# EnzoCording/FleetRL

Hardware: NVIDIA B200
Metric: EV-steps/sec (higher is better)
Workload: dtype f64

## Files before the change

fleetrl_b200/csrc/fleetstep.cu:

```cuda
#include <cuda_runtime.h>
#include <math.h>
#include <stdint.h>
#include <stdio.h>
#include <stdlib.h>
#include <string.h>

#include <string>
#include <vector>

#include "fleetstep.h"

namespace {

constexpr int kThreads = 256;
constexpr int kMinCtasPerSm = 4;
constexpr int kStatStripes = 64;
constexpr int kNQ = 5;
enum { Q_REWARD = 0, Q_CASH, Q_ATH, Q_MISS, Q_NVIOL };

constexpr uint32_t TF_TRIGGER = 1u;
constexpr uint32_t TF_LUNCH = 2u;

constexpr int EF_FROZEN = 1, EF_DONE = 2, EF_TRIGGER = 4, EF_LUNCH = 8, EF_RESET = 16;

// ... 166 lines not shown

template <bool kNorm, bool kAux>
__device__ __forceinline__ void write_ev_obs(const StepParams& p, float* __restrict__ o, int n, double soc, float hl,
                                             const EvRec& rec, bool flip) {
    const int N = p.N;
    o[n] = (float)soc;
    o[N + n] = kNorm ? (float)((double)hl / p.max_tl) : hl;
    if (kAux) {
        float4 ax = make_float4(rec.tt, rec.cl, rec.hn, rec.lax);
        if (flip) ax = aux_on_the_fly<kNorm>(0.9, rec.sr, rec.tl, rec.there, p.lc_batt_cap, p.hn_den, p.max_soc, p.max_hn);
        float* a = o + 2 * N + p.Ha;
        a[n] = (float)rec.there;
        a[N + n] = ax.x;
        a[2 * N + n] = ax.y;
        a[3 * N + n] = ax.z;
        a[4 * N + n] = ax.w;
    }
}

template <bool kAux>
__device__ __forceinline__ int hdr_pos(int Ha, int N, int q) {
    return q < Ha ? 2 * N + q : 2 * N + Ha + (kAux ? 5 * N : 0) + (q - Ha);
}
template <bool kAux>
__device__ __forceinline__ void copy_hdr(const StepParams& p, float* __restrict__ o, int n, int t) {
    const float* __restrict__ h = p.hdr + (size_t)t * p.hdr_stride;
    for (int q = n; q < (kAux ? p.Ha + p.Hb : p.Ha); q += p.N) o[hdr_pos<kAux>(p.Ha, p.N, q)] = __ldg(h + q);
}

template <bool kNorm, bool kAux>
__device__ __forceinline__ void reset_slot(const StepParams& p, int e, int n, int t0, float* obs_row, bool reinit_deg) {
    const size_t i = (size_t)e * p.N + n;
    const EvRec rec = load_rec(&p.ev_rec[(size_t)t0 * p.N + n]);
    bool flip = false;
    if (reinit_deg) {
        p.rf_len[i] = 1; p.fd_cyc[i] = 0; p.life[i] = 1 - p.init_soh;
        p.tflip[i] = 0;
    } else if (*p.n_flips != 0) {
        flip = p.tflip[i] != 0;
    }
    const double tgt = flip ? 0.9 : p.target;
    const double soh = 1.0 * p.init_soh;
    const double cap = soh * p.cap0;
    double soc = rec.sr;
    const float hl = rec.tl;
    const double time_needed = (tgt - soc) * cap / p.P;
    if (hl > 0.f && p.min_lax * time_needed > (double)hl) soc = tgt - (time_needed * p.P / cap) / p.min_lax;
    const double sdeg = (soc == 0) ? p.def_soc : soc;
    p.soc[i] = soc;
    p.hl[i] = hl;
    p.soh[i] = soh;
    p.hist[((size_t)e * p.R + 0) * p.N + n] = sdeg;
    if (p.rf_on) {
        const int slot = p.rf_ext[i];
        if (slot >= 0) { atomicExch(&p.ext_owner[slot], -1); p.rf_ext[i] = -1; }
        p.rf_stack[i * (size_t)p.rf_S] = sdeg;
        p.rf_dc[i] = 1u;
        p.rf_acc[i] = make_double2(0.0, 0.0);
    }
    if (obs_row) {
        write_ev_obs<kNorm, kAux>(p, obs_row, n, soc, hl, rec, flip);
        copy_hdr<kAux>(p, obs_row, n, t0);
    }
}

#ifdef POST_TIMING
__device__ unsigned long long g_post_clk[16];
#ifdef POST_TIMING_EVAL_ONLY
#define PT_ON(c_) (c_)
#else
#define PT_ON(c_) true
#endif
#define PT_START2(k_, c_) long long _pt = clock64(); const bool _pt_on = (k_) && PT_ON(c_)
#define PT_START(c_) PT_START2(true, c_)
#define PT_MARK(k) do { if (threadIdx.x == 0 && _pt_on) { const long long _c = clock64(); atomicAdd(&g_post_clk[k], (unsigned long long)(_c - _pt)); _pt = _c; } } while (0)
#define PT_COUNT(k, n) do { if (threadIdx.x == 0 && _pt_on) atomicAdd(&g_post_clk[k], (unsigned long long)(n)); } while (0)
#else
#define PT_START(c_) do {} while (0)
#define PT_START2(k_, c_) do {} while (0)
#define PT_MARK(k) do {} while (0)
#define PT_COUNT(k, n) do {} while (0)
#endif
constexpr int kPostThreads = 64;
constexpr int kRfBatch = 8;
constexpr int kRfQueue = 12;
constexpr int kRfPend = 8;
constexpr int kPostMinCtas = 8;

__device__ __forceinline__ double sei_cycle_stress(double range, double count, double mean, double s_temp) {
    const double k_sigma = 1.04, sigma_ref = 0.5, kd1 = 1.4E5, kd2 = -5.01E-1, kd3 = -1.23E5;
    double eff = range * count;
    eff = eff < 0 ? 0 : (eff > 1 ? 1 : eff);
    const double s_dod = 1.0 / (kd1 * exp(kd2 * log(eff)) + kd3);
    const double s_soc = exp(k_sigma * (mean - sigma_ref));
    return s_dod * s_soc * s_temp;
}

__global__ void debug_stress_kernel(const double* eff, const double* mean, double* out, int n) {
    const int i = blockIdx.x * blockDim.x + threadIdx.x;
    if (i < n) out[i] = sei_cycle_stress(eff[i], 1.0, mean[i], 1.0);
}

__device__ __noinline__ int rf_ext_alloc(const StepParams& p, size_t vid) {
    const unsigned P = (unsigned)p.rf_P;
    if (P == 0) return -1;
    unsigned q = (unsigned)(mix64((unsigned long long)vid) % P);
    for (unsigned k = 0; k < P; k++) {
        if (atomicCAS(&p.ext_owner[q], -1, (int)vid) == -1) return (int)q;
        if (++q == P) q = 0;
    }
    return -1;
}

__device__ __forceinline__ double empirical_eval(double dt, double evse, double old_soc, double new_soc) {
    const double avg_soc = (old_soc + new_soc) / 2;
    const double cs[3] = {0, 40, 90};
    const double ca[3] = {0.0065, 0.0293, 0.065};
    int best = 0;
    double bd = fabs(cs[0] - avg_soc);
#pragma unroll
    for (int k = 1; k < 3; k++) {
        const double d = fabs(cs[k] - avg_soc);
        if (d < bd) { bd = d; best = k; }
    }
    const double cal = ca[best] * dt / 8760;
    const double dod = fabs(new_soc - old_soc);
    const double cyc = (evse <= 22.0) ? dod * 0.000125 / 2 : dod * 0.000167 / 2;
    return cal + cyc;
}

__device__ __forceinline__ void cp_async_commit() { asm volatile("cp.async.commit_group;" ::: "memory"); }
template <int kPending>
__device__ __forceinline__ void cp_async_wait_group() { asm volatile("cp.async.wait_group %0;" :: "n"(kPending) : "memory"); }
__device__ __forceinline__ void cp_async4_hint(uint32_t sdst, const void* gsrc, uint64_t pol) {
    asm volatile("cp.async.ca.shared.global.L2::cache_hint [%0], [%1], 4, %2;" :: "r"(sdst), "l"(gsrc), "l"(pol) : "memory");
}
__device__ __forceinline__ void cp_async8_hint(uint32_t sdst, const void* gsrc, uint64_t pol) {
    asm volatile("cp.async.ca.shared.global.L2::cache_hint [%0], [%1], 8, %2;" :: "r"(sdst), "l"(gsrc), "l"(pol) : "memory");
}
__device__ __forceinline__ void cp_async16_hint(uint32_t sdst, const void* gsrc, uint64_t pol) {
    asm volatile("cp.async.cg.shared.global.L2::cache_hint [%0], [%1], 16, %2;" :: "r"(sdst), "l"(gsrc), "l"(pol) : "memory");
}
__device__ __forceinline__ uint64_t l2_evict_first_policy() {
    uint64_t pol;
    asm volatile("createpolicy.fractional.L2::evict_first.b64 %0, 1.0;" : "=l"(pol));
    return pol;
}

__device__ __forceinline__ double sei_fade_update(const StepParams& p, size_t i, int len, int m, int rfl, double msum,
                                                  double fsum, bool big, double s_temp, bool& consumed) {
    const double alpha_sei = 5.75E-2, beta_sei = 121, k_sigma = 1.04, sigma_ref = 0.5, k_dt = 4.14E-10;
    double deg = 0;
    consumed = false;
    p.n_cycles[i] = m;
    if (m > rfl) {
        const double battery_age = (double)(len - 1) * p.dt * 3600;
        const double mean_soc_cal = msum / (double)m;
        if (big) atomicOr(p.err_flags, 4u);
        const double fd_cal = (k_dt * battery_age) * exp(k_sigma * (mean_soc_cal - sigma_ref)) * s_temp;
        const double fd_cyc = p.fd_cyc[i] + fsum;
        p.fd_cyc[i] = fd_cyc;
        const double fd = fd_cyc + fd_cal;
        const double l_old = p.life[i];
        double new_l;
        if (p.init_soh == 1.0) {
            new_l = 1 - alpha_sei * exp(-beta_sei * fd) - (1 - alpha_sei) * exp(-fd);
            if (new_l < 0) atomicOr(p.err_flags, 2u);
        } else {
// ... 8 lines not shown
    p.soh[i] = p.soh[i] - deg;
    return deg;
}

__device__ __noinline__ double rf_vehicle_slow(const StepParams& p, int e, int n, int k_done, int k_now, bool evaluate,
                                               double s_temp) {
    const int N = p.N, S = p.rf_S, X = p.rf_X, Rm = p.Rm;
    const size_t i = (size_t)e * N + n;
    const unsigned int dc = p.rf_dc[i];
    int depth = (int)(dc & 0xffffu), c = (int)(dc >> 16);
    double2 acc = p.rf_acc[i];
    int slot = p.rf_ext[i];
    const int rfl = p.rf_len[i];
    const double* hcol = p.hist + (size_t)e * p.RN + n;
    double* stk = p.rf_stack + i * (size_t)S;
    double* ext = slot >= 0 ? p.ext_val + (size_t)slot * X : nullptr;
#define RF_GET(s_) ((s_) < S ? stk[(s_)] : ext[(s_) - S])
#define RF_PUT(s_, v_) do { if ((s_) < S) stk[(s_)] = (v_); else ext[(s_) - S] = (v_); } while (0)
    bool bad = false, big = false;
    double x_cur = hcol[(size_t)(k_done & Rm) * N];
    double dsg = x_cur - RF_GET(depth - 1);
    for (int r = k_done + 1; r <= k_now; r++) {
        const double x_next = hcol[(size_t)(r & Rm) * N];
        if (x_next == x_cur) continue;
        const double d = x_next - x_cur;
        if ((dsg < 0 && d > 0) || (dsg > 0 && d < 0)) {
            if (depth >= S && !ext) {
                slot = (depth < S + X) ? rf_ext_alloc(p, i) : -1;
                if (slot >= 0) ext = p.ext_val + (size_t)slot * X;
            }
            if (depth >= S + X || (depth >= S && !ext)) bad = true;
            else {
                RF_PUT(depth, x_cur); depth++;
                while (depth >= 3) {
                    const double x3 = RF_GET(depth - 1), x2 = RF_GET(depth - 2), x1 = RF_GET(depth - 3);
                    if (fabs(x3 - x2) < fabs(x2 - x1)) break;
                    const double range = fabs(x1 - x2), mean = 0.5 * (x1 + x2);
                    const bool half = depth == 3;
                    acc.x += mean;
                    if (c >= rfl - 1) { acc.y += sei_cycle_stress(range, half ? 0.5 : 1.0, mean, s_temp); big = big || range > 5; }
                    c++;
                    if (half) { RF_PUT(0, x2); RF_PUT(1, x3); depth = 2; }
                    else { RF_PUT(depth - 3, x3); depth -= 2; }
                }
            }
        }
        dsg = d; x_cur = x_next;
    }
    if (bad) atomicOr(p.err_flags, 8u);
    double deg = 0;
    if (evaluate) {
        const int len = k_now + 1;
        int m = c, h = depth, lo = 0;
        double msum = acc.x, fs = 0;
        if (len >= 3) {
            auto prov = [&](double xa, double xb, double cnt, bool last) {
                const double range = fabs(xa - xb), mean = 0.5 * (xa + xb);
                msum += mean;
                if (!last && m >= rfl - 1) { fs += sei_cycle_stress(range, cnt, mean, s_temp); big = big || range > 5; }
                m++;
            };
            while (h - lo >= 2) {
                const double x2 = RF_GET(h - 1), x1 = RF_GET(h - 2);
                if (fabs(x_cur - x2) < fabs(x2 - x1)) break;
                if (h - lo == 2) { prov(x1, x2, 0.5, false); lo++; }
                else { prov(x1, x2, 1.0, false); h -= 2; }
            }
            for (int k = lo; k + 1 < h; k++) prov(RF_GET(k), RF_GET(k + 1), 0.5, false);
            prov(RF_GET(h - 1), x_cur, 0.5, true);
        }
        bool consumed;
        deg = sei_fade_update(p, i, len, m, rfl, msum, acc.y + fs, big, s_temp, consumed);
        if (consumed) acc.y = 0;
    }
#undef RF_GET
#undef RF_PUT
    if (slot >= 0 && depth <= S) { atomicExch(&p.ext_owner[slot], -1); slot = -1; }
    p.rf_dc[i] = (unsigned int)depth | ((unsigned int)c << 16);
    p.rf_acc[i] = acc;
    p.rf_ext[i] = slot;
    return deg;
}

template <int kT, bool kEval>
__device__ __forceinline__ double rf_vehicle(const StepParams& p, int e, int n, bool active, int k_done, int k_now,
                                             bool evaluate, double s_temp, double* __restrict__ smcol,
                                             double* __restrict__ qcol, double2* __restrict__ pcol) {
    const unsigned full = 0xffffffffu;
    const int N = p.N, S = p.rf_S, Rm = p.Rm;
    const double inf = __longlong_as_double(0x7ff0000000000000ll);
    const size_t i = (size_t)e * N + (active ? n : 0);
    const double* __restrict__ hcol = p.hist + (size_t)e * p.RN + (active ? n : 0);
    double* __restrict__ stk = p.rf_stack + i * (size_t)S;
    int depth = 1, c = 0, rflm1 = 0;
    double2 acc = make_double2(0.0, 0.0);
    double x_cur = 0;
    if (active) {
        const unsigned int dc = p.rf_dc[i];
        acc = p.rf_acc[i];
        rflm1 = p.rf_len[i] - 1;
        x_cur = __ldcs(hcol + (size_t)(k_done & Rm) * N);
        for (int s = 0; s < S; s += 2) {
            const double2 v2 = *reinterpret_cast<const double2*>(stk + s);
            smcol[s * kT] = v2.x; smcol[(s + 1) * kT] = v2.y;
        }
        depth = (int)(dc & 0xffffu); c = (int)(dc >> 16);
    }
    bool slow = active && depth > S;
    bool live = active && !slow;
    PT_START2(kEval, evaluate);
    double t1 = 0, t2 = 0, Y = inf;
    if (live) {
        t1 = smcol[(depth - 1) * kT];
        if (depth >= 2) { t2 = smcol[(depth - 2) * kT]; Y = fabs(t1 - t2); }
    }
    double dsg = live ? x_cur - t1 : 0.0;
    bool big = false;
    int np = 0;
    bool has_item = false;
    double item_eff = 0, item_mean = 0;
#define RF_APPEND(target_)                                                                     \
    do {                                                                                       \
        if (has_item) { pcol[np * kT] = make_double2(item_eff, item_mean); np++; has_item = false; } \
        if (__any_sync(full, np == kRfPend)) RF_DRAIN(target_);                                \
    } while (0)
#define RF_DRAIN(target_)                                                                      \
    do {                                                                                       \
        const int m_ = __reduce_max_sync(full, np);                                            \
        for (int k_ = 0; k_ < m_; k_ += 2) {                                                   \
            const double2 i0_ = pcol[min(k_, kRfPend - 1) * kT];                     \
            const double2 i1_ = pcol[min(k_ + 1, kRfPend - 1) * kT];                 \
            const double s0_ = sei_cycle_stress(i0_.x, 1.0, i0_.y, s_temp);                    \
            const double s1_ = sei_cycle_stress(i1_.x, 1.0, i1_.y, s_temp);                    \
            if (k_ < np) (target_) += s0_;                                                     \
            if (k_ + 1 < np) (target_) += s1_;                                                 \
        }                                                                                      \
        np = 0;                                                                                \
    } while (0)

    int nq = 0;
    for (int r0 = k_done + 1; ; r0 += kRfBatch) {
        const bool more = r0 <= k_now;
        if (__any_sync(full, more ? nq > kRfQueue - kRfBatch : nq > 0)) {
            PT_MARK(2);
            int q = 0;
            while (__any_sync(full, q < nq)) {
                const bool act = q < nq;
                const double v = qcol[min(q, kRfQueue - 1) * kT];
                const double X = fabs(v - t1);
                const bool lt = X < Y, two = depth == 2;
                const bool closing = act && !lt;
                const bool full_c = closing && !two;
                const bool consume = act && (lt || two);
                const bool push = act && lt;
                if (push && depth >= S) { slow = true; live = false; nq = 0; }
                else {
                    const double mean = 0.5 * (t2 + t1);
                    acc.x += closing ? mean : 0.0;
                    has_item = closing && c >= rflm1;
                    item_eff = two ? 0.5 * Y : Y; item_mean = mean;
                    big = big || (closing && Y > 5);
                    c += closing ? 1 : 0;
                    if (push) smcol[max(depth - 2, 0) * kT] = t2;
                    depth += push ? 1 : (full_c ? -2 : 0);
                    const double s1 = smcol[max(depth - 1, 0) * kT], s2 = smcol[max(depth - 2, 0) * kT];
                    t2 = consume ? t1 : (full_c ? s2 : t2);
                    t1 = consume ? v : (full_c ? s1 : t1);
                    Y = consume ? X : (full_c ? (depth >= 2 ? fabs(t1 - t2) : inf) : Y);
                    q += consume ? 1 : 0;
                }
                PT_COUNT(10, 1);
                RF_APPEND(acc.y);
            }
            nq = 0;
            PT_MARK(3);
        }
        if (!__any_sync(full, more)) break;
        double xb[kRfBatch];
#pragma unroll
        for (int u = 0; u < kRfBatch; u++) xb[u] = __ldcs(hcol + (size_t)(min(r0 + u, k_now) & Rm) * N);
#pragma unroll
        for (int u = 0; u < kRfBatch; u++) {
            const double d = xb[u] - x_cur;
            const bool flip = live && (dsg * d < 0);
            if (flip) { qcol[nq * kT] = x_cur; nq++; }
            dsg = (d != 0) ? d : dsg;
            x_cur = live ? xb[u] : x_cur;
        }
    }
    RF_DRAIN(acc.y);
    PT_MARK(4);
    if (live) { smcol[(depth - 1) * kT] = t1; if (depth >= 2) smcol[(depth - 2) * kT] = t2; }

    double deg = 0;
    if (kEval && evaluate) {
        const int len = k_now + 1;
        int m = c, h = depth, lo = 0, k = 0;
        double msum = acc.x, fs = 0;
        int phase = (live && len >= 3) ? 0 : 2;
        while (__any_sync(full, phase < 2)) {
            if (phase == 0) {
                bool closed = false;
                if (h - lo >= 2) {
                    const double x2 = smcol[(h - 1) * kT], x1 = smcol[(h - 2) * kT];
                    const double yy = fabs(x2 - x1);
                    if (!(fabs(x_cur - x2) < yy)) {
                        closed = true;
                        const double mean = 0.5 * (x1 + x2);
                        msum += mean;
                        if (m >= rflm1) { has_item = true; item_eff = h - lo == 2 ? 0.5 * yy : yy; item_mean = mean; big = big || yy > 5; }
                        m++;
                        if (h - lo == 2) lo++; else h -= 2;
                    }
                }
                if (!closed) { phase = 1; k = lo; }
            } else if (phase == 1) {
                const double xa = smcol[k * kT], xb2 = (k + 1 < h) ? smcol[(k + 1) * kT] : x_cur;
                const double mean = 0.5 * (xa + xb2);
                msum += mean;
                if (k + 1 < h) {
                    const double rg = fabs(xa - xb2);
                    if (m >= rflm1) { has_item = true; item_eff = 0.5 * rg; item_mean = mean; big = big || rg > 5; }
                    k++;
                } else phase = 2;
                m++;
            }
            RF_APPEND(fs);
        }
        RF_DRAIN(fs);
        if (live) {
            bool consumed;
            deg = sei_fade_update(p, i, len, m, rflm1 + 1, msum, acc.y + fs, big, s_temp, consumed);
            if (consumed) acc.y = 0;
        }
    }
#undef RF_APPEND
#undef RF_DRAIN
    PT_MARK(5);
    if (live) {
        for (int s = 0; s < S; s += 2)
            *reinterpret_cast<double2*>(stk + s) = make_double2(smcol[s * kT], smcol[(s + 1) * kT]);
        p.rf_dc[i] = (unsigned int)depth | ((unsigned int)c << 16);
        p.rf_acc[i] = acc;
    }
    PT_MARK(6);
    if (slow) deg = rf_vehicle_slow(p, e, n, k_done, k_now, evaluate, s_temp);
    PT_MARK(7);
    return deg;
}

__device__ __forceinline__ void bulk_store_s2g(void* gdst, const void* ssrc, uint32_t bytes) {
    asm volatile("fence.proxy.async.shared::cta;" ::: "memory");
    asm volatile("cp.async.bulk.global.shared::cta.bulk_group [%0], [%1], %2;"
                 :: "l"(gdst), "r"((uint32_t)__cvta_generic_to_shared(ssrc)), "r"(bytes) : "memory");
    asm volatile("cp.async.bulk.commit_group;" ::: "memory");
}
__device__ __forceinline__ void bulk_store_s2g_nofence(void* gdst, const void* ssrc, uint32_t bytes) {
    uint64_t pol;
    asm volatile("createpolicy.fractional.L2::evict_first.b64 %0, 1.0;" : "=l"(pol));
    asm volatile("cp.async.bulk.global.shared::cta.bulk_group.L2::cache_hint [%0], [%1], %2, %3;"
                 :: "l"(gdst), "r"((uint32_t)__cvta_generic_to_shared(ssrc)), "r"(bytes), "l"(pol) : "memory");
    asm volatile("cp.async.bulk.commit_group;" ::: "memory");
}
__device__ __forceinline__ void thread_store_range(float* gdst, const float* ssrc, int nfl) {
    int head = (int)(((16u - (unsigned)((uintptr_t)gdst & 15u)) & 15u) >> 2);
    head = head < nfl ? head : nfl;
    const int mid = (nfl - head) & ~3;
    for (int k = 0; k < head; k++) gdst[k] = ssrc[k];
    if (mid > 0) bulk_store_s2g_nofence(gdst + head, ssrc + head, (uint32_t)mid * 4u);
    for (int k = head + mid; k < nfl; k++) gdst[k] = ssrc[k];
}
__device__ __forceinline__ void bulk_store_wait_read() {
    asm volatile("cp.async.bulk.wait_group.read 0;" ::: "memory");
}

__device__ __forceinline__ void ev_slot_step(const StepParams& p, const EnvS& es, size_t i, bool flip, double a, double soh,
                                             double sr, float ntl, int there, double& soc, float& hl, double& sdeg,
                                             double& q_rew, double& q_cash, double& q_ath, double& q_miss, double& q_nviol,
                                             double& q_en) {
    const double tgt = flip ? 0.9 : p.target;
    const double cap = soh * p.cap0;
    double c_cr = 0, c_dr = 0, c_inv = 0, c_oc = 0, c_dep = 0, c_cost = 0, c_rev = 0, c_miss = 0, c_nviol = 0;
    double num = 0;
    if (a >= 0) {
        const double dem = (tgt - soc) * cap;
        const double req = p.P * a * p.dt;
        if (req * p.eta_c > dem) {
            const double d = req - dem;
            const double pen = p.pen_oc * (d * d);
            c_oc = pen > p.clip_oc ? pen : p.clip_oc;
        }
        double en = 0;
        if (there == 1) en = fmin(dem / p.eta_c, req);
        else if (fabs(a) > 0.05) c_inv = p.pen_inv * (a * a);
        num = en * p.eta_c;
        q_en = en;
        double ge = en - es.pv_share;
        ge = ge > 0 ? ge : 0;
        c_cost = ge * es.S * p.mult;
        c_cr = es.F_cr * ge;
    } else if (a < 0) {
        const double left = -1 * soc * cap;
        const double req = p.P * a * p.dt;
        if (req * p.eta_d < left && there != 0) {
            const double d = left - req;
            c_oc = p.pen_oc * (d * d);
        }
        double en = 0.0;
        if (there == 1) en = fmax(left, req);
        else if (fabs(a) > 0.05) c_inv = p.pen_inv * (a * a);
        num = en;
        q_en = en;
        c_rev = -1 * en * es.Rfac;
        c_dr = es.F_dr * en;
    } else {
        q_en = 0;
        atomicOr(p.err_flags, 1u);
    }
    q_ath = a * (double)there;
    if (num != 0) soc = soc + num / cap;

    if (hl != 0.f && ntl == 0.f) {
        const double tg = (p.is_ct && (es.flags & EF_LUNCH)) ? p.target_lunch : tgt;
        const double diff = tg - soc;
// ... 516 lines not shown
        PF_MARK(7);
#endif

        double q_rew = 0, q_cash = 0, q_ath = 0, q_miss = 0, q_nviol = 0;
        double o_soc = 0, o_sdeg = 0, o_en = 0;
        float o_hl = 0.f;
        size_t o_hist = 0;
        if (active) {
            const EnvS& es = envs[b];
            float* orow = obs_tile + b * D;
            const size_t i = (size_t)tile * cstride + j;
            const int t1 = min(es.t + 1, p.T - 1);
            const int k = es.t - es.t_start;
            const EvRec rec = decode_rec(reinterpret_cast<const int4*>(stp + kPfStR0)[j],
                                         reinterpret_cast<const int4*>(stp + kPfStR1)[j]);
            o_soc = reinterpret_cast<const double*>(stp + kPfStSoc)[j];
            o_sdeg = reinterpret_cast<const double*>(stp + kPfStSdeg)[j];
            const double soh = reinterpret_cast<const double*>(stp + kPfStSoh)[j];
            o_hl = reinterpret_cast<const float*>(stp + kPfStHl)[j];
            const double a = (double)reinterpret_cast<const float*>(stp + kPfStA32)[j];
            float hv0 = 0.f;
            if (n < H) hv0 = reinterpret_cast<const float*>(stp + kPfStHv)[j];
            const bool flip = s_have_flips && p.tflip[i] != 0;
            ev_slot_step(p, es, i, flip, a, soh, rec.sr, rec.tl, rec.there_prev, o_soc, o_hl, o_sdeg, q_rew, q_cash, q_ath,
                         q_miss, q_nviol, o_en);
            o_hist = (size_t)(unsigned)tile * p.pf_tile_hist + hist_slot + (unsigned)(((k + 1) & p.Rm) * N);
            write_ev_obs<kNorm, kAux>(p, orow, n, o_soc, o_hl, rec, flip);
            if (n < H) orow[hpos] = hv0;
            for (int q = n + N; q < H; q += N)
                orow[hdr_pos<kAux>(p.Ha, N, q)] = ld_keep_f32(p.hdr + (size_t)t1 * p.hdr_stride + q, keep);
        }
        if (pair) {
            q_rew += __shfl_xor_sync(0xffffffffu, q_rew, 1);
            q_cash += __shfl_xor_sync(0xffffffffu, q_cash, 1);
            q_ath += __shfl_xor_sync(0xffffffffu, q_ath, 1);
            q_miss += __shfl_xor_sync(0xffffffffu, q_miss, 1);
            q_nviol += __shfl_xor_sync(0xffffffffu, q_nviol, 1);
        }
        if (active && !(pair && (j & 1))) {
            const int cj = pair ? (j >> 1) : j;
            contrib[Q_REWARD * cslots + cj] = q_rew;
            contrib[Q_CASH * cslots + cj] = q_cash;
            contrib[Q_ATH * cslots + cj] = q_ath;
            contrib[Q_MISS * cslots + cj] = q_miss;
            contrib[Q_NVIOL * cslots + cj] = q_nviol;
        }
        PF_MARK(1);
        asm volatile("fence.proxy.async.shared::cta;" ::: "memory");
        mbar_arrive(&bar_done[buf]);
        PF_MARK(5);
        PF_TRACE(tid >> 5, it, 3);
        if (active) {
            const size_t i = (size_t)tile * cstride + j;
            __stcs(p.soc + i, o_soc);
            __stcs(p.hl + i, o_hl);
            __stcs(p.hist + o_hist, o_sdeg);
            if (kLog) __stcs(p.charge_log + i, o_en);
        }
        PF_MARK(6);
        issue_copies(tile + kPfStages * G, ev_next, stg);
        PF_MARK(3);
        PF_TRACE(tid >> 5, it, 4);
        if (++stg == kPfStages) stg = 0;
        if (++ebuf == kPfEnvs) { ebuf = 0; ph_env ^= 1u; }
        if (++buf == kPfOut) { buf = 0; if (it >= kPfOut) ph_free ^= 1u; }
    }
    PF_FLUSH(8);
}

__device__ __forceinline__ void post_finish_lists(const StepParams& p) {
    if (threadIdx.x == 0) {
        __threadfence();
        const unsigned int d = atomicAdd(p.wl_done, 1u);
        if (d == gridDim.x - 1) {
            p.wl_count[0] = 0; p.wl_count[1] = 0; p.wl_count[2] = 0; p.wl_count[3] = 0; p.wl_count[4] = 0;
            *p.wl_done = 0;
        }
    }
}

template <bool kNorm, bool kAux, int kT>
__global__ void __launch_bounds__(kT, kT == 32 ? 2 * kPostMinCtas : kPostMinCtas) fleet_post_kernel(const __grid_constant__ StepParams p) {
    extern __shared__ __align__(16) unsigned char smem_raw[];
    double* sm_stack = reinterpret_cast<double*>(smem_raw);
    double* sm_queue = sm_stack + (size_t)p.rf_S * kT;
    double2* sm_pend = reinterpret_cast<double2*>(sm_queue + (size_t)kRfQueue * kT);
    __shared__ int s_w;
    __shared__ int2 s_ent;
    __shared__ int4 s_ev;
    __shared__ double s_deg;
    const int tid = threadIdx.x, N = p.N;
    const int n_front = p.wl_count[0];
    const int count = n_front + p.wl_count[2];
    const double temp_ref = 25, k_temp = 6.93E-2;
    const double s_temp = exp(k_temp * (p.temperature - temp_ref) * ((temp_ref + 273.15) / (p.temperature + 273.15)));

    const int chunks = p.post_chunks, cv = p.post_cv;
    const int items = count * chunks;
    if (tid == 0) {
        s_w = blockIdx.x; s_deg = 0;
        if (s_w < items) { s_ent = wl_fetch(p, s_w / chunks, n_front); s_ev = p.env4[s_ent.x]; }
    }
    for (;;) {
        __syncthreads();
        const int item = s_w;
        if (item >= items) break;
        const int w = item / chunks, chunk = item - w * chunks;
        const int2 ent = s_ent;
        const int e = ent.x, wf = ent.y;
        const int4 ev = s_ev;
        const int k_now = ev.x - ev.y;
        const int n = chunk * cv + tid;
        const bool mine = tid < cv && n < N;
        int w_next = 0;
        int2 ent_next = make_int2(0, 0);
        int4 ev_next = make_int4(0, 0, 0, 0);
        if (tid == 0) {
            w_next = atomicAdd(p.wl_count + 1, 1) + (int)gridDim.x;
            if (w_next < items) { ent_next = wl_fetch(p, w_next / chunks, n_front); ev_next = p.env4[ent_next.x]; }
        }
        PT_START((wf & WL_TRIGGER) != 0);
        PT_COUNT(11, 1);
        if (p.rf_on && (wf & (WL_TRIGGER | WL_FLUSH))) {
            PT_COUNT(12, 1);
            const double deg = rf_vehicle<kT, true>(p, e, n, mine, ev.w, k_now, (wf & WL_TRIGGER) != 0, s_temp, sm_stack + tid,
                                              sm_queue + tid, sm_pend + tid);
            if (deg != 0) atomicAdd(&s_deg, deg);
        } else if ((wf & WL_TRIGGER) && mine) {
            const double* hbase = p.hist + (size_t)e * p.RN;
            const size_t ii = (size_t)e * N + n;
            double deg = 0;
            if (k_now >= 1) deg = empirical_eval(p.dt, p.evse, hbase[(size_t)((k_now - 1) & p.Rm) * N + n], hbase[(size_t)(k_now & p.Rm) * N + n]);
            p.n_cycles[ii] = 0;
            p.last_deg[ii] = deg;
            p.soh[ii] = p.soh[ii] - deg;
            if (deg != 0) atomicAdd(&s_deg, deg);
        }
        __syncthreads();
        PT_MARK(8);
        if (tid == 0 && s_deg != 0)
            atomicAdd(p.stats + (size_t)(w % kStatStripes) * FLEET_S__COUNT + FLEET_S_DEGRADATION, s_deg);
        int t0 = 0;
        if (wf & WL_RESET) {
            PT_COUNT(13, 1);
            t0 = episode_start(p, p.next_start, e, ev.z);
            if (mine) reset_slot<kNorm, kAux>(p, e, n, t0, p.obs ? p.obs + (size_t)e * p.D : nullptr, !p.carry);
            PT_MARK(14);
        }
        if (tid == 0) {
            bool last = true;
            if (chunks > 1) {
                __threadfence();
                last = atomicAdd(p.wl_chunks + w, 1) == chunks - 1;
                if (last) p.wl_chunks[w] = 0;
            }
            if (last) {
                if (wf & WL_RESET) {
                    begin_episode(p, e, t0, ev.z);
                } else if (p.rf_on) {
                    p.env4[e] = make_int4(ev.x, ev.y, ev.z, k_now);
                }
            }
        }
        __syncthreads();
        PT_MARK(9);
        if (tid == 0) { s_w = w_next; s_ent = ent_next; s_ev = ev_next; s_deg = 0; }
    }

    const int n_flush = p.wl_count[3];
    if (n_flush > 0) {
        const unsigned full = 0xffffffffu;
        const int lane = tid & 31;
        const int vehicles = n_flush * N;
        const int units = (vehicles + 31) >> 5;
        for (;;) {
            int u = 0;
            if (lane == 0) u = atomicAdd(p.wl_count + 4, 1);
            u = __shfl_sync(full, u, 0);
            if (u >= units) break;
#ifdef POST_TIMING
            const long long pt_u = clock64();
#endif
            const int v = (u << 5) + lane;
            const bool active = v < vehicles;
            int4 fe = make_int4(0, 0, 0, 0);
            int n = 0;
            if (active) {
                const int f = v / N;
                n = v - f * N;
                fe = p.wl_flush[f];
            }
            if (active && n == N - 1) p.env4[fe.x].w = fe.z;
            rf_vehicle<kT, false>(p, fe.x, n, active, fe.y, fe.z, false, s_temp, sm_stack + tid, sm_queue + tid, sm_pend + tid);
#ifdef POST_TIMING
            if (lane == 0) { atomicAdd(&g_post_clk[15], 1ull); atomicAdd(&g_post_clk[0], (unsigned long long)(clock64() - pt_u)); }
#endif
        }
    }
    __syncthreads();
    post_finish_lists(p);
}

template <bool kNorm, bool kAux>
__global__ void __launch_bounds__(kThreads) fleet_reset_kernel(const StepParams p) {
    const int N = p.N, B = p.B;
    const int e0 = blockIdx.x * B;
    const int nb = min(B, p.E - e0);
    const int nslots = nb * N;
    for (int j = threadIdx.x; j < nslots; j += kThreads) {
        const int b = j / N, n = j - b * N;
        const int e = e0 + b;
        if (p.mask && !p.mask[e]) continue;
        const int t0 = episode_start(p, p.start_idx, e, p.env4[e].z);
        reset_slot<kNorm, kAux>(p, e, n, t0, p.obs ? p.obs + (size_t)e * p.D : nullptr, !p.carry);
    }
    __syncthreads();
    if (threadIdx.x < nb) {
        const int e = e0 + threadIdx.x;
        if (!(p.mask && !p.mask[e])) {
            const int ep_count = p.env4[e].z;
            begin_episode(p, e, episode_start(p, p.start_idx, e, ep_count), ep_count);
        }
    }
}

__global__ void init_state_kernel(StepParams p) {
    const size_t i = (size_t)blockIdx.x * blockDim.x + threadIdx.x;
    const size_t EN = (size_t)p.E * p.N;
    if (i < EN) {
        p.soc[i] = 0; p.hl[i] = 0; p.soh[i] = p.init_soh;
        p.rf_len[i] = 1; p.fd_cyc[i] = 0; p.life[i] = 1 - p.init_soh; p.n_cycles[i] = 0; p.last_deg[i] = 0;
        p.tflip[i] = 0;
        if (p.rf_on) { p.rf_dc[i] = 1u; p.rf_acc[i] = make_double2(0.0, 0.0); p.rf_ext[i] = -1; }
    }
    if (i < (size_t)p.E) p.env4[i] = make_int4(0, 0, 0, 0);
}

__global__ void policy_kernel(StepParams p, int policy, int ch_hour, int ch_minute, int max_h, const uint16_t* __restrict__ tod,
                              const int2* __restrict__ st_in, int2* __restrict__ st_out, float* __restrict__ actions) {
    const size_t i = (size_t)blockIdx.x * blockDim.x + threadIdx.x;
    if (i >= (size_t)p.E * p.N) return;
    const int e = (int)(i / p.N), n = (int)(i - (size_t)e * p.N);
    const int t = min(p.env4[e].x, p.T - 1);
    float a = 1.f;
    if (policy != FLEET_POLICY_UNCONTROLLED) {
        const EvRec rec = load_rec(&p.ev_rec[(size_t)t * p.N + n]);
        const bool flip = (*p.n_flips != 0) && p.tflip[i] != 0;
        const double tgt = flip ? 0.9 : p.target;
        const double cl = tgt * (double)rec.there - rec.sr;
        const double hn = cl * p.lc_batt_cap / p.hn_den;
        double d = hn / ((double)rec.tl + 0.001);
        d = d < 0 ? 0 : (d > 1 ? 1 : d);
        if (policy == FLEET_POLICY_DISTRIBUTED) {
            a = (float)d;
        } else {
            const int hour = tod[t] / 60, minute = tod[t] % 60;
            int2 st = st_in[e];
            if (p.is_ct && hour >= 11 && hour <= 14) {
                a = (float)d;
            } else {
                if ((ch_hour <= hour && ch_minute <= minute) || st.x) {
                    if (!st.x) st.y = t;
                    st.x = 1;
                    a = 1.f;
                } else {
                    a = 0.f;
                }
                if (st.x && (double)(t - st.y) * p.dt > (double)max_h) st.x = 0;
            }
            if (n == 0) st_out[e] = st;
        }
    }
    actions[i] = a;
}

__global__ void gather_field_kernel(StepParams p, int field, void* dst) {
// ... 590 lines not shown
        rfX = env_int("FLEETSTEP_RF_EXT", 52);
        if (rfS + rfX > c.episode_steps + 1) rfX = c.episode_steps + 1 - rfS;
        if (rfX < 0) rfX = 0;
        rfP = rfX > 0 ? env_int("FLEETSTEP_RF_EXT_SLOTS", (int)(EN / 128 < 64 ? 64 : (EN / 128 > (1u << 20) ? (1u << 20) : EN / 128))) : 0;
        if (EN >= 0x7fffffffull) return fail(h, FLEET_E_INVALID, "num_envs * num_evs must be below 2^31");
    }
    if ((rc = dev_alloc(h, &p.env4, (size_t)E))) return rc;
    if ((rc = dev_alloc(h, &p.soc, EN))) return rc;
    if ((rc = dev_alloc(h, &p.hl, EN))) return rc;
    if ((rc = dev_alloc(h, &p.soh, EN))) return rc;
    if ((rc = dev_alloc(h, &p.hist, EN * (size_t)R))) return rc;
    if ((rc = dev_alloc(h, &p.tflip, EN))) return rc;
    if ((rc = dev_alloc(h, &p.n_flips, (size_t)4))) return rc;
    if ((rc = dev_alloc(h, &p.env_f64, (size_t)EF__COUNT * E))) return rc;
    if ((rc = dev_alloc(h, &p.rf_len, EN))) return rc;
    if ((rc = dev_alloc(h, &p.fd_cyc, EN))) return rc;
    if ((rc = dev_alloc(h, &p.life, EN))) return rc;
    if ((rc = dev_alloc(h, &p.n_cycles, EN))) return rc;
    if ((rc = dev_alloc(h, &p.last_deg, EN))) return rc;
    if ((rc = dev_alloc(h, &p.stats, (size_t)kStatStripes * FLEET_S__COUNT))) return rc;
    if ((rc = dev_alloc(h, &p.err_flags, (size_t)4))) return rc;
    if ((rc = dev_alloc(h, &p.wl, (size_t)E))) return rc;
    if ((rc = dev_alloc(h, &p.wl_flush, (size_t)E))) return rc;
    if (rf_on) {
        if ((rc = dev_alloc(h, &p.rf_stack, EN * (size_t)rfS))) return rc;
        if ((rc = dev_alloc(h, &p.rf_dc, EN))) return rc;
        if ((rc = dev_alloc(h, &p.rf_acc, EN))) return rc;
        if ((rc = dev_alloc(h, &p.rf_ext, EN))) return rc;
        if ((rc = dev_alloc(h, &p.ext_owner, (size_t)(rfP > 0 ? rfP : 1)))) return rc;
        if ((rc = dev_alloc(h, &p.ext_val, (size_t)(rfP > 0 ? rfP : 1) * (size_t)(rfX > 0 ? rfX : 1), false))) return rc;
        CUDA_TRY(h, cudaMemset(p.ext_owner, 0xff, sizeof(int) * (size_t)(rfP > 0 ? rfP : 1)));
    }
    if ((rc = dev_alloc(h, &p.wl_count, (size_t)8))) return rc;
    if ((rc = dev_alloc(h, &p.wl_done, (size_t)4))) return rc;

    p.rf_on = rf_on ? 1 : 0; p.rf_S = rfS; p.rf_X = rfX; p.rf_P = rfP;
    p.E = E; p.N = N; p.T = T; p.R = R; p.Rm = R - 1; p.L = c.episode_steps; p.D = h->D; p.Ha = Ha; p.Hb = Hb; p.hdr_stride = hdr_stride;
    p.B = N >= kThreads ? 1 : kThreads / N;
    p.RN = (unsigned long long)R * (unsigned long long)N;
    p.is_ct = c.is_caretaker; p.calc_deg = c.calc_degradation; p.deg_mode = c.deg_mode; p.carry = c.carry_degradation_state;
    p.auto_reset = c.auto_reset; p.start_lo = c.start_lo; p.start_hi = c.start_hi; p.seed = c.seed;
    p.env_id_offset = env_id_offset;
    p.dt = c.dt; p.dt_f = (float)c.dt;
    p.P = c.obc_max_power < c.evse_max_power ? c.obc_max_power : c.evse_max_power;
    p.eta_c = c.charging_eff; p.eta_d = c.discharging_eff; p.mult = c.variable_multiplier; p.cap0 = c.init_battery_cap;
    p.target = 1.0 * c.target_soc; p.target_lunch = c.target_soc_lunch; p.eps = c.soc_eps; p.def_soc = c.def_soc;
    p.min_lax = c.min_laxity; p.pen_inv = c.penalty_invalid_action; p.pen_oc = c.penalty_overcharging;
    p.clip_oc = c.clip_overcharging; p.pen_ovl = c.penalty_overloading; p.full_reward = c.fully_charged_reward;
    p.evse = c.evse_max_power; p.grid = c.grid_connection; p.init_soh = c.init_soh; p.lc_batt_cap = c.lc_batt_cap;
    p.hn_den = c.evse_max_power * c.charging_eff;
    p.price_mult = c.price_multiplier; p.temperature = c.temperature;
    p.max_tl = c.max_time_left; p.max_soc = c.target_soc;
    p.max_hn = (c.target_soc * c.init_battery_cap) / (c.evse_max_power * c.charging_eff);
    p.ev_rec = d_rec; p.step_row = d_rows; p.hdr = d_hdr;
    {
        std::vector<uint16_t> tod((size_t)T);
        for (int tt = 0; tt < T; tt++) tod[tt] = (uint16_t)(tb->hour[tt] * 60 + tb->minute[tt]);
        if ((rc = dev_alloc(h, &h->tod, (size_t)T, false))) return rc;
        CUDA_TRY(h, cudaMemcpy(h->tod, tod.data(), tod.size() * sizeof(uint16_t), cudaMemcpyHostToDevice));
    }

    p.n_magic = (unsigned int)((0x100000000ull + (unsigned long long)N - 1) / (unsigned long long)N);
    {
        const unsigned long long Hh = (unsigned long long)(Ha + Hb > 0 ? Ha + Hb : 1);
        p.h_magic = (unsigned int)((0x100000000ull + Hh - 1) / Hh);
    }
    p.off_contrib = (int)smem_envs_bytes(p.B);
    p.off_obs = (int)smem_obs_offset(p.B, N);
    p.bulk_ok = ((p.B * h->D) % 4 == 0) ? 1 : 0;

    size_t sm = smem_step_bytes(p.B, N, h->D);
    if ((int64_t)sm > (int64_t)h->max_smem_optin) {
        char buf[256];
        snprintf(buf, sizeof buf, "step kernel needs %zu bytes of shared memory (N=%d, D=%d) but the device allows %d", sm, N,
                 h->D, h->max_smem_optin);
        return fail(h, FLEET_E_INVALID, buf);
    }
    h->num_sms = prop.multiProcessorCount;
    h->need_post = (c.calc_degradation || c.auto_reset) ? 1 : 0;
    h->post_threads = N <= 32 ? 32 : 64;
    p.post_chunks = (N + h->post_threads - 1) / h->post_threads;
    p.post_cv = (N + p.post_chunks - 1) / p.post_chunks;
    if (p.post_chunks > 1 && (rc = dev_alloc(h, &p.wl_chunks, (size_t)E))) return rc;
    h->smem_post = align16((size_t)(rfS + kRfQueue + 2 * kRfPend) * h->post_threads * 8);
    if ((int64_t)h->smem_post > (int64_t)h->max_smem_optin) return fail(h, FLEET_E_INVALID, "rf_stack_depth does not fit the post kernel's shared memory");
    {
        int per_sm = 1;
        CUDA_TRY(h, cudaFuncSetAttribute(pick_post(h), cudaFuncAttributeMaxDynamicSharedMemorySize, (int)h->smem_post));
        CUDA_TRY(h, cudaOccupancyMaxActiveBlocksPerMultiprocessor(&per_sm, pick_post(h), h->post_threads, h->smem_post));
        if (per_sm < 1) per_sm = 1;
        const int64_t g = (int64_t)h->num_sms * per_sm;
        h->grid_post = (int)(g < E ? g : E);
        const int cap = env_int("FLEETSTEP_POST_GRID", 0);
        if (cap > 0 && cap < h->grid_post) h->grid_post = cap;
    }
    h->smem_step = sm;
    {
        const char* zc = getenv("FLEETSTEP_HOST_ZEROCOPY");
        h->host_zerocopy = (zc && atoi(zc) == 0) ? 0 : 1;
    }
    {
        const char* force = getenv("FLEETSTEP_KERNEL");
        const bool want = !force || strcmp(force, "pf") == 0;
        const int pfB = kPfSlots / N;
        if (want && c.auto_reset && N >= 8 && pfB >= 1 && pfB <= 32) {
            const size_t smpf = pf_smem_bytes(pfB, N, h->D);
            int per_sm = 0;
            if ((int64_t)smpf <= (int64_t)h->max_smem_optin &&
                cudaFuncSetAttribute(pick_pf(h, false), cudaFuncAttributeMaxDynamicSharedMemorySize, (int)smpf) == cudaSuccess &&
                cudaFuncSetAttribute(pick_pf(h, true), cudaFuncAttributeMaxDynamicSharedMemorySize, (int)smpf) == cudaSuccess &&
                cudaOccupancyMaxActiveBlocksPerMultiprocessor(&per_sm, pick_pf(h, true), kPfThreads, smpf) == cudaSuccess && per_sm >= 1) {
                h->smem_pf = smpf;
                const int ntiles = (E + pfB - 1) / pfB;
                p.pf_B = pfB;
                p.pf_bulk = 1;
                p.pf_ntiles = ntiles;
                p.pf_tile_hist = (unsigned int)((size_t)pfB * p.RN);
                p.pf_pair = (N & 1) ? 0 : 1;
                p.pf_cslots = pf_contrib_slots(pfB, N);
                p.pf_cper = p.pf_pair ? N / 2 : N;
                p.pf_envs_b = (int)align16((size_t)pfB * sizeof(EnvS));
                p.pf_contrib_b = (int)align16((size_t)kNQ * p.pf_cslots * 8);
                p.pf_obs_b = (int)align16((size_t)pfB * h->D * 4 + 12);
                p.pf_off_contrib = kPfEnvs * p.pf_envs_b;
                p.pf_off_sums = p.pf_off_contrib + kPfOut * p.pf_contrib_b;
                p.pf_off_obs = p.pf_off_sums + 2 * (int)align16((size_t)kNQ * pfB * 8);
                p.pf_off_stage = (int)align16((size_t)p.pf_off_obs + (size_t)kPfOut * p.pf_obs_b);
                const int g = prop.multiProcessorCount * per_sm;
                h->grid_pf = g < ntiles ? g : ntiles;
                const int cap = env_int("FLEETSTEP_PF_GRID", 0);
                if (cap > 0 && cap < h->grid_pf) h->grid_pf = cap;
                h->use_pf = 1;
            }
            cudaGetLastError();
        }
        if (force && strcmp(force, "pf") == 0 && !h->use_pf)
            return fail(h, FLEET_E_INVALID, "FLEETSTEP_KERNEL=pf requested but the configuration does not qualify (needs auto_reset, 8 <= N <= 256)");
    }
    h->grid = (E + p.B - 1) / p.B;
    CUDA_TRY(h, cudaFuncSetAttribute(pick_step(h), cudaFuncAttributeMaxDynamicSharedMemorySize, (int)sm));

    init_state_kernel<<<(unsigned)((EN > (size_t)E ? EN : (size_t)E) + 255) / 256, 256>>>(p);
    h->launches++;
    CUDA_TRY(h, cudaGetLastError());
    CUDA_TRY(h, cudaDeviceSynchronize());
    return FLEET_OK;
}

int fleet_reset(FleetHandle* h, const int32_t* start_idx_dev, const uint8_t* mask_dev, float* obs_dev, void* stream) {
    if (!h) return FLEET_E_INVALID;
    CUDA_TRY(h, cudaSetDevice(h->device));
    StepParams p = h->p;
    p.start_idx = start_idx_dev; p.mask = mask_dev; p.obs = obs_dev;
    pick_reset(h)<<<h->grid, kThreads, 0, (cudaStream_t)stream>>>(p);
    h->launches++;
    if (h->log_n) fleet_log_launch(h, p, 1, (cudaStream_t)stream);
    CUDA_TRY(h, cudaGetLastError());
    return FLEET_OK;
}

int fleet_step(FleetHandle* h, const float* actions_dev, float* obs_dev, float* reward_dev, uint8_t* done_dev,
               float* terminal_obs_dev, void* stream) {
    if (!h) return FLEET_E_INVALID;
    if (!actions_dev) return fail(h, FLEET_E_INVALID, "actions_dev is NULL");
    CUDA_TRY(h, cudaSetDevice(h->device));
    StepParams p = h->p;
    p.actions = actions_dev; p.obs = obs_dev; p.reward = reward_dev; p.done = done_dev; p.terminal_obs = terminal_obs_dev;
// ... 203 lines not shown
```

Baseline: 24.59 billion.

## Stream rainflow history spans via cp.async and prefetch next flush work unit

Rainflow processing now loads the vehicle's stack and up to 16 history rows into shared memory with cp.async and an L2 evict-first hint, instead of strided direct loads in batches of 8. Turning-point detection runs over the shared span, and the detected points reuse the span buffer in place of a separate queue. Stack entries are stored as double2 with lookahead reads of the next stack values. In the flush loop, the next work-unit claim and its metadata fetch overlap the current vehicle's async loads through a pre-wait callback. This restructures the memory schedule and adds complexity, and the larger span buffer raises shared-memory use and can lower occupancy.

```diff
diff --git a/fleetrl_b200/csrc/fleetstep.cu b/fleetrl_b200/csrc/fleetstep.cu
--- a/fleetrl_b200/csrc/fleetstep.cu
+++ b/fleetrl_b200/csrc/fleetstep.cu
@@ -272,8 +272,8 @@
 #define PT_COUNT(k, n) do {} while (0)
 #endif
 constexpr int kPostThreads = 64;
+constexpr int kRfSpan = 16;
 constexpr int kRfBatch = 8;
-constexpr int kRfQueue = 12;
 constexpr int kRfPend = 8;
 constexpr int kPostMinCtas = 8;
 
@@ -448,37 +448,46 @@
     return deg;
 }
 
-template <int kT, bool kEval>
+template <int kT, bool kEval, typename PreWait>
 __device__ __forceinline__ double rf_vehicle(const StepParams& p, int e, int n, bool active, int k_done, int k_now,
-                                             bool evaluate, double s_temp, double* __restrict__ smcol,
-                                             double* __restrict__ qcol, double2* __restrict__ pcol) {
+                                             bool evaluate, double s_temp, double2* __restrict__ smcol,
+                                             double* __restrict__ span, double2* __restrict__ pcol, PreWait&& pre_wait) {
     const unsigned full = 0xffffffffu;
     const int N = p.N, S = p.rf_S, Rm = p.Rm;
     const double inf = __longlong_as_double(0x7ff0000000000000ll);
     const size_t i = (size_t)e * N + (active ? n : 0);
     const double* __restrict__ hcol = p.hist + (size_t)e * p.RN + (active ? n : 0);
     double* __restrict__ stk = p.rf_stack + i * (size_t)S;
+#define RF_STK(s_) (reinterpret_cast<double*>(smcol + ((s_) >> 1) * kT)[(s_) & 1])
+    const uint64_t pol = l2_evict_first_policy();
+    const uint32_t span_s = (uint32_t)__cvta_generic_to_shared(span);
+    auto load_span = [&](int r0, int nr) {
+        for (int j = 0; j < nr; j++)
+            cp_async8_hint(span_s + (uint32_t)(j * kT * 8), hcol + (size_t)((r0 + j) & Rm) * N, pol);
+        cp_async_commit();
+    };
+    PT_START2(kEval, evaluate);
+    int nr = active ? max(1, min(kRfSpan, k_now - k_done + 1)) : 0;
+    if (active) {
+        const uint32_t sm_s = (uint32_t)__cvta_generic_to_shared(smcol);
+        for (int s = 0; s < S; s += 2) cp_async16_hint(sm_s + (uint32_t)((s >> 1) * kT * 16), stk + s, pol);
+    }
+    load_span(k_done, nr);
     int depth = 1, c = 0, rflm1 = 0;
     double2 acc = make_double2(0.0, 0.0);
-    double x_cur = 0;
-    if (active) {
-        const unsigned int dc = p.rf_dc[i];
-        acc = p.rf_acc[i];
-        rflm1 = p.rf_len[i] - 1;
-        x_cur = __ldcs(hcol + (size_t)(k_done & Rm) * N);
-        for (int s = 0; s < S; s += 2) {
-            const double2 v2 = *reinterpret_cast<const double2*>(stk + s);
-            smcol[s * kT] = v2.x; smcol[(s + 1) * kT] = v2.y;
-        }
-        depth = (int)(dc & 0xffffu); c = (int)(dc >> 16);
-    }
+    unsigned int dc = 1;
+    if (active) { dc = p.rf_dc[i]; acc = p.rf_acc[i]; rflm1 = p.rf_len[i] - 1; }
+    pre_wait();
+    cp_async_wait_group<0>();
+    PT_MARK(1);
+    depth = (int)(dc & 0xffffu); c = (int)(dc >> 16);
     bool slow = active && depth > S;
     bool live = active && !slow;
-    PT_START2(kEval, evaluate);
+    double x_cur = active ? span[0] : 0.0;
     double t1 = 0, t2 = 0, Y = inf;
     if (live) {
-        t1 = smcol[(depth - 1) * kT];
-        if (depth >= 2) { t2 = smcol[(depth - 2) * kT]; Y = fabs(t1 - t2); }
+        t1 = RF_STK(depth - 1);
+        if (depth >= 2) { t2 = RF_STK(depth - 2); Y = fabs(t1 - t2); }
     }
     double dsg = live ? x_cur - t1 : 0.0;
     bool big = false;
@@ -504,15 +513,30 @@
         np = 0;                                                                                \
     } while (0)
 
-    int nq = 0;
-    for (int r0 = k_done + 1; ; r0 += kRfBatch) {
-        const bool more = r0 <= k_now;
-        if (__any_sync(full, more ? nq > kRfQueue - kRfBatch : nq > 0)) {
-            PT_MARK(2);
+    for (int r0 = k_done, j0 = 1; ; ) {
+        int nq = 0;
+        const int m = __reduce_max_sync(full, nr);
+        for (int j = j0; j < m; j += kRfBatch) {
+            double xb[kRfBatch];
+#pragma unroll
+            for (int u = 0; u < kRfBatch; u++) xb[u] = span[min(j + u, kRfSpan - 1) * kT];
+#pragma unroll
+            for (int u = 0; u < kRfBatch; u++) {
+                const double xv = j + u < nr ? xb[u] : x_cur;
+                const double d = xv - x_cur;
+                const bool flip = live && (dsg * d < 0);
+                if (flip) { span[nq * kT] = x_cur; nq++; }
+                dsg = (d != 0) ? d : dsg;
+                x_cur = live ? xv : x_cur;
+            }
+        }
+        PT_MARK(2);
+        {
             int q = 0;
+            double v = span[0];
             while (__any_sync(full, q < nq)) {
                 const bool act = q < nq;
-                const double v = qcol[min(q, kRfQueue - 1) * kT];
+                const double b1 = RF_STK(max(depth - 3, 0)), b2 = RF_STK(max(depth - 4, 0));
                 const double X = fabs(v - t1);
                 const bool lt = X < Y, two = depth == 2;
                 const bool closing = act && !lt;
@@ -527,36 +551,29 @@
                     item_eff = two ? 0.5 * Y : Y; item_mean = mean;
                     big = big || (closing && Y > 5);
                     c += closing ? 1 : 0;
-                    if (push) smcol[max(depth - 2, 0) * kT] = t2;
+                    if (push) RF_STK(max(depth - 2, 0)) = t2;
                     depth += push ? 1 : (full_c ? -2 : 0);
-                    const double s1 = smcol[max(depth - 1, 0) * kT], s2 = smcol[max(depth - 2, 0) * kT];
-                    t2 = consume ? t1 : (full_c ? s2 : t2);
-                    t1 = consume ? v : (full_c ? s1 : t1);
+                    t2 = consume ? t1 : (full_c ? b2 : t2);
+                    t1 = consume ? v : (full_c ? b1 : t1);
                     Y = consume ? X : (full_c ? (depth >= 2 ? fabs(t1 - t2) : inf) : Y);
                     q += consume ? 1 : 0;
+                    v = span[min(q, kRfSpan - 1) * kT];
                 }
                 PT_COUNT(10, 1);
                 RF_APPEND(acc.y);
             }
-            nq = 0;
             PT_MARK(3);
         }
-        if (!__any_sync(full, more)) break;
-        double xb[kRfBatch];
-#pragma unroll
-        for (int u = 0; u < kRfBatch; u++) xb[u] = __ldcs(hcol + (size_t)(min(r0 + u, k_now) & Rm) * N);
-#pragma unroll
-        for (int u = 0; u < kRfBatch; u++) {
-            const double d = xb[u] - x_cur;
-            const bool flip = live && (dsg * d < 0);
-            if (flip) { qcol[nq * kT] = x_cur; nq++; }
-            dsg = (d != 0) ? d : dsg;
-            x_cur = live ? xb[u] : x_cur;
-        }
+        r0 += kRfSpan; j0 = 0;
+        nr = active ? min(kRfSpan, k_now - r0 + 1) : 0;
+        if (!__any_sync(full, nr > 0)) break;
+        load_span(r0, nr);
+        cp_async_wait_group<0>();
+        PT_MARK(1);
     }
     RF_DRAIN(acc.y);
     PT_MARK(4);
-    if (live) { smcol[(depth - 1) * kT] = t1; if (depth >= 2) smcol[(depth - 2) * kT] = t2; }
+    if (live) { RF_STK(depth - 1) = t1; if (depth >= 2) RF_STK(depth - 2) = t2; }
 
     double deg = 0;
     if (kEval && evaluate) {
@@ -568,7 +585,7 @@
             if (phase == 0) {
                 bool closed = false;
                 if (h - lo >= 2) {
-                    const double x2 = smcol[(h - 1) * kT], x1 = smcol[(h - 2) * kT];
+                    const double x2 = RF_STK(h - 1), x1 = RF_STK(h - 2);
                     const double yy = fabs(x2 - x1);
                     if (!(fabs(x_cur - x2) < yy)) {
                         closed = true;
@@ -581,7 +598,7 @@
                 }
                 if (!closed) { phase = 1; k = lo; }
             } else if (phase == 1) {
-                const double xa = smcol[k * kT], xb2 = (k + 1 < h) ? smcol[(k + 1) * kT] : x_cur;
+                const double xa = RF_STK(k), xb2 = (k + 1 < h) ? RF_STK(k + 1) : x_cur;
                 const double mean = 0.5 * (xa + xb2);
                 msum += mean;
                 if (k + 1 < h) {
@@ -602,10 +619,11 @@
     }
 #undef RF_APPEND
 #undef RF_DRAIN
+#undef RF_STK
     PT_MARK(5);
     if (live) {
         for (int s = 0; s < S; s += 2)
-            *reinterpret_cast<double2*>(stk + s) = make_double2(smcol[s * kT], smcol[(s + 1) * kT]);
+            *reinterpret_cast<double2*>(stk + s) = smcol[(s >> 1) * kT];
         p.rf_dc[i] = (unsigned int)depth | ((unsigned int)c << 16);
         p.rf_acc[i] = acc;
     }
@@ -1288,9 +1306,9 @@
 template <bool kNorm, bool kAux, int kT>
 __global__ void __launch_bounds__(kT, kT == 32 ? 2 * kPostMinCtas : kPostMinCtas) fleet_post_kernel(const __grid_constant__ StepParams p) {
     extern __shared__ __align__(16) unsigned char smem_raw[];
-    double* sm_stack = reinterpret_cast<double*>(smem_raw);
-    double* sm_queue = sm_stack + (size_t)p.rf_S * kT;
-    double2* sm_pend = reinterpret_cast<double2*>(sm_queue + (size_t)kRfQueue * kT);
+    double2* sm_stack = reinterpret_cast<double2*>(smem_raw);
+    double* sm_span = reinterpret_cast<double*>(sm_stack + (size_t)(p.rf_S / 2) * kT);
+    double2* sm_pend = reinterpret_cast<double2*>(sm_span + (size_t)kRfSpan * kT);
     __shared__ int s_w;
     __shared__ int2 s_ent;
     __shared__ int4 s_ev;
@@ -1330,7 +1348,7 @@
         if (p.rf_on && (wf & (WL_TRIGGER | WL_FLUSH))) {
             PT_COUNT(12, 1);
             const double deg = rf_vehicle<kT, true>(p, e, n, mine, ev.w, k_now, (wf & WL_TRIGGER) != 0, s_temp, sm_stack + tid,
-                                              sm_queue + tid, sm_pend + tid);
+                                                    sm_span + tid, sm_pend + tid, [] {});
             if (deg != 0) atomicAdd(&s_deg, deg);
         } else if ((wf & WL_TRIGGER) && mine) {
             const double* hbase = p.hist + (size_t)e * p.RN;
@@ -1379,25 +1397,35 @@
         const int lane = tid & 31;
         const int vehicles = n_flush * N;
         const int units = (vehicles + 31) >> 5;
-        for (;;) {
-            int u = 0;
-            if (lane == 0) u = atomicAdd(p.wl_count + 4, 1);
-            u = __shfl_sync(full, u, 0);
-            if (u >= units) break;
-#ifdef POST_TIMING
-            const long long pt_u = clock64();
-#endif
+        auto fetch = [&](int u, int& n, int4& fe) {
             const int v = (u << 5) + lane;
-            const bool active = v < vehicles;
-            int4 fe = make_int4(0, 0, 0, 0);
-            int n = 0;
-            if (active) {
+            n = 0; fe = make_int4(0, 0, 0, 0);
+            if (u < units && v < vehicles) {
                 const int f = v / N;
                 n = v - f * N;
                 fe = p.wl_flush[f];
             }
+        };
+        int u = 0;
+        if (lane == 0) u = atomicAdd(p.wl_count + 4, 1);
+        u = __shfl_sync(full, u, 0);
+        int n; int4 fe;
+        fetch(u, n, fe);
+        while (u < units) {
+#ifdef POST_TIMING
+            const long long pt_u = clock64();
+#endif
+            int claim = 0;
+            if (lane == 0) claim = atomicAdd(p.wl_count + 4, 1);
+            int u_next = units, n_next; int4 fe_next;
+            const bool active = (u << 5) + lane < vehicles;
             if (active && n == N - 1) p.env4[fe.x].w = fe.z;
-            rf_vehicle<kT, false>(p, fe.x, n, active, fe.y, fe.z, false, s_temp, sm_stack + tid, sm_queue + tid, sm_pend + tid);
+            rf_vehicle<kT, false>(p, fe.x, n, active, fe.y, fe.z, false, s_temp, sm_stack + tid, sm_span + tid, sm_pend + tid,
+                                  [&] {
+                                      u_next = __shfl_sync(full, claim, 0);
+                                      fetch(u_next, n_next, fe_next);
+                                  });
+            u = u_next; n = n_next; fe = fe_next;
 #ifdef POST_TIMING
             if (lane == 0) { atomicAdd(&g_post_clk[15], 1ull); atomicAdd(&g_post_clk[0], (unsigned long long)(clock64() - pt_u)); }
 #endif
@@ -2154,7 +2182,7 @@
     p.post_chunks = (N + h->post_threads - 1) / h->post_threads;
     p.post_cv = (N + p.post_chunks - 1) / p.post_chunks;
     if (p.post_chunks > 1 && (rc = dev_alloc(h, &p.wl_chunks, (size_t)E))) return rc;
-    h->smem_post = align16((size_t)(rfS + kRfQueue + 2 * kRfPend) * h->post_threads * 8);
+    h->smem_post = align16((size_t)(rfS + kRfSpan + 2 * kRfPend) * h->post_threads * 8);
     if ((int64_t)h->smem_post > (int64_t)h->max_smem_optin) return fail(h, FLEET_E_INVALID, "rf_stack_depth does not fit the post kernel's shared memory");
     {
         int per_sm = 1;
```

Result: slower. 24.14 billion, median of 6 (-1.8%).
